# vklyukin/nf_distillation

Measured on NVIDIA B200. Metric: kd_train_samples_per_sec, higher is better.
Workload: dtype bf16

## Files before the change

### include/nfk.h

```cpp
#ifndef NFK_H_
#define NFK_H_

#ifdef __cplusplus
extern "C" {
#endif

#define NFK_OK 0
#define NFK_ERR_SHAPE (-1)
#define NFK_ERR_ALIGN (-2)
#define NFK_ERR_ARG (-3)
#define NFK_ERR_LAUNCH (-4)
#define NFK_ERR_DRIVER (-5)

#define NFK_EPI_F32 0
#define NFK_EPI_BIAS_RELU_BF16 1
#define NFK_EPI_MASK_BF16 2

int nfk_version(void);

int nfk_gemm_nt_bf16(const void* A, long long lda, const void* B, long long ldb, int M, int N, int K, int epi,
                     void* out, long long ldo, const float* bias, const void* aux, long long ldaux, float* colsum,
                     void* stream);

int nfk_gemm_set_prof(void* buf);
// ... 48 lines not shown
                      const float* l2, const float* w3, const float* b3, const float* l3, int cin, int hid, int cout,
                      int K1p, int K3p, void* B1, void* B1T, void* B2, void* B2T, void* B3, void* B3T, float* bias1,
                      float* bias2, float* bias3, int with_transposed, void* stream);

int nfk_coupling_prep_bwd(const float* w1, const float* b1, const float* l1, const float* w2, const float* b2,
                          const float* l2, const float* w3, const float* b3, const float* l3, int cin, int hid,
                          int cout, int K1p, int K3p, const float* dB1, const float* dbias1, const float* dB2,
                          const float* dbias2, const float* dB3, const float* dbias3, float* dw1, float* db1,
                          float* dl1, float* dw2, float* db2, float* dl2, float* dw3, float* db3, float* dl3,
                          void* stream);

int nfk_affine1x1_fwd(const float* x, const float* Wf, const float* bf, const float* sl, float* y, void* col,
                      int K1p, const float* ld_in, float* ld_out, int B, int C, int H, int W, void* stream);

int nfk_coupling_fwd(const float* P, int K3p, const float* bias3, float* y, float* hsave, float* ld, int B, int C,
                     int H, int W, int reverse, void* stream);

int nfk_coupling_bwd(const float* g_out, const float* g_ld, const float* z_out, const float* hsave, float* dy,
                     void* dhcol, int K3p, float* dbias3, int B, int C, int H, int W, void* stream);

int nfk_affine1x1_bwd(const float* dy, const float* dcol, int K1p, const float* x, const float* Wf, float* dx,
                      float* dWf, float* dbf, int B, int C, int H, int W, void* stream);

int nfk_coupling_inv_bwd(const float* g_zc, const float* g_ld, const float* zc, const float* hsave, float* dz,
                         void* dhcol, int K3p, float* dbias3, int B, int C, int H, int W, void* stream);

int nfk_col2im_add(const float* dcol, int K1p, float* dz, int B, int C, int H, int W, void* stream);

int nfk_split2d_fwd(const float* x, const float* w, const float* bias, const float* logs, float* z1_out, float* ld,
                    int B, int C, int H, int W, void* stream);
int nfk_split2d_rev(const float* z1, const float* w, const float* bias, const float* logs, const float* eps,
                    float temperature, float* out, int B, int C, int H, int W, void* stream);
int nfk_split2d_bwd(const float* x, const float* w, const float* bias, const float* logs, const float* g_z1,
                    const float* g_ld, float* dx, float* dw, float* dbias, float* dlogs, int B, int C, int H, int W,
                    void* stream);
int nfk_split2d_squeeze_fwd(const float* x, const float* w, const float* bias, const float* logs, float* z1_out,
                            float* z1_sq_out, float* ld, int B, int C, int H, int W, void* stream);
int nfk_split2d_squeeze_bwd(const float* x, const float* w, const float* bias, const float* logs, const float* g_z1,
                            const float* g_z1_sq, const float* g_ld, float* dx, float* dw, float* dbias, float* dlogs,
                            int B, int C, int H, int W, void* stream);
int nfk_dequant_squeeze(const void* src, int src_is_u8, int n_bits, const float* noise, float* x_out, float* sq_out,
                        int B, int C, int H, int W, void* stream);
int nfk_prior_bpd_fwd(const float* z, const float* mean, const float* logs, const float* logdet, int B, int n,
                      float scale, float* out, void* stream);
int nfk_prior_bpd_bwd(const float* z, const float* mean, const float* logs, const float* g_bpd, int B, int n,
                      float scale, float* dz, float* dlogdet, void* stream);
int nfk_kd_mse_fwd(const float* s, const float* t, int B, int n, float scale, float* acc, void* stream);
int nfk_kd_mse_bwd(const float* s, const float* t, const float* g, int B, int n, float scale, float* ds,
                   int accumulate, void* stream);

int nfk_pconv_coupling_supported(int C, int H, int W, int hid);
int nfk_pconv_coupling_fwd(const void* h2, const void* B3, int K3p, const float* bias3, float* y, float* hsave,
                           float* ld, int B, int C, int H, int W, int hid, int reverse, void* stream);

int nfk_flow1d_supported(int D, int Cc, int hid, int training);
int nfk_flow1d_sizes(int D, int Cc, int hid, int* total_fwd, int* total_bwd, int* total_grad, int* n_act,
                     int* offsets);
int nfk_flow1d_pack(const float* Wf, const float* bf, const float* const* w, const float* const* b, int D, int Cc,
                    int hid, float* PF, float* PB, void* stream);
int nfk_flow1d_fwd(const float* x, const float* cond, const float* PF, const float* sl, float* y, const float* ld_in,
                   float* ld_out, float* acts, int B, int D, int Cc, int hid, int reverse, void* stream);
int nfk_flow1d_bwd(const float* x_in, const float* cond, const float* acts, const float* PB, const float* y_out,
                   const float* g_out, const float* g_ld, float* dx, float* G, int B, int D, int Cc, int hid,
                   int reverse, void* stream);
int nfk_affine_rows(const float* x, const float* Wf, const float* bf, const float* sl, float* y, const float* ld_in,
                    float* ld_out, int B, int D, float pixels, void* stream);

int nfk_gemm_nt_bf16_ranged(const void* A, long long lda, const void* B, long long ldb, int M, int N, int K, int epi,
                            void* out, long long ldo, const float* bias, const void* aux, long long ldaux,
                            float* colsum, int bn, const int* kb_begin, const int* kb_end, void* stream);

int nfk_made_prep(const float* w1, const float* w2, const float* w3, const int* deg1, const int* deg2, int D, int H,
                  int Dp, int N3p, void* B1, void* B1T, void* B2, void* B2T, void* B3, void* B3T, int with_t,
                  void* stream);
int nfk_made_prep_bwd(const float* dB1, const float* dB2, const float* dB3, const int* deg1, const int* deg2, int D,
                      int H, int Dp, float* dw1, float* dw2, float* dw3, void* stream);
int nfk_rows_to_bf16(const float* x, int B, int D, int Dp, void* xb, void* stream);
int nfk_made_affine_fwd(const float* x, const float* out, int N3p, float* u, void* ub, int Dp, const float* ld_in,
                        float* ld_out, int B, int D, int flip, void* stream);
int nfk_made_affine_bwd(const float* x, const float* out, int N3p, const float* g_u, const float* g_ld, float* dx,
                        void* dout, float* db3, int B, int D, int flip, void* stream);
int nfk_made_inv_update(float* x, void* xb, int Dp, const float* u_in, const float* out, int N3p, const float* ld_in,
                        float* ld_out, int B, int D, int i, int flip, int last, void* stream);
int nfk_made_inverse_resident_supported(int D, int H, int Dp);
int nfk_made_inverse_push_supported(int D, int H, int Dp, int N3p);
int nfk_made_inverse_jobs(const int* cnt1, const int* cnt2, int D, int H, int Dp, int N3p, int push, int* jobs,
                          int cap);
int nfk_made_inverse_pack(const int* jobs, int njobs, const void* B1, const void* B2, const void* B3, int N3p, int D,
                          int H, int Dp, int push, void* wstream, void* stream);
int nfk_made_inverse_resident(const float* u_in, const void* wstream, const float* b1, const float* b2,
                              const float* b3, const int* jobs, int njobs, int push, int N3p, float* x,
                              const float* ld_in, float* ld_out, int B, int D, int H, int Dp, int flip, int mtiles,
                              void* stream);

int nfk_cnet_set_prof(void* buf);
int nfk_cnet_fwd_fused(const void* col, int K1p, const void* B1, const void* B2, const float* bias1,
                       const float* bias2, void* h1, void* h2, void* mask1, void* mask2, long long ldmask, int M,
                       int hid, void* stream);
int nfk_cnet_bwd_fused(const void* dhcol, int K3p, const void* B3T, const void* B2T, const void* mask_h2,
                       const void* mask_h1, long long ldmask, void* dpre2, void* dpre1, float* dbias2, float* dbias1,
                       int M, int hid, void* stream);
int nfk_cnet_fwd_fused_ranged(const void* col, int K1p, const void* B1, const void* B2, const float* bias1,
                              const float* bias2, void* h1, void* h2, void* mask1, void* mask2, long long ldmask,
                              int M, int hid, int kb2_end_half0, void* stream);

#define NFK_LOSS_MAX_LEVELS 8
// ... 37 lines not shown
```

### nf_distillation_b200/_lib.py

```python
from __future__ import annotations

import ctypes
import os

from . import build as _build

_c = ctypes
_vp, _i, _ll, _f = _c.c_void_p, _c.c_int, _c.c_longlong, _c.c_float

ERRORS = {
    -1: "NFK_ERR_SHAPE (unsupported / inconsistent sizes)",
    -2: "NFK_ERR_ALIGN (pointer or leading dimension not 16-byte aligned)",
    -3: "NFK_ERR_ARG (missing / invalid argument)",
    -4: "NFK_ERR_LAUNCH (CUDA launch failure)",
    -5: "NFK_ERR_DRIVER (tensor-map encode failure)",
}



class InvconvItem(_c.Structure):
    _fields_ = [(n, _vp) for n in ("an_bias", "an_logs", "lower", "upper", "log_s", "p", "sign_s", "weight")] + \
               [("C", _i), ("reverse", _i), ("transpose", _i)] + \
               [(n, _vp) for n in ("outW", "outb", "out_sl")]

# ... 16 lines not shown
               [(n, _vp) for n in ("dw1", "db1", "dl1", "dw2", "db2", "dl2", "dw3", "db3", "dl3")]


NFK_LOSS_MAX_LEVELS = 8


class LossLevels(_c.Structure):
    _fields_ = [("s", _vp * NFK_LOSS_MAX_LEVELS), ("t", _vp * NFK_LOSS_MAX_LEVELS), ("ds", _vp * NFK_LOSS_MAX_LEVELS),
                ("n", _i * NFK_LOSS_MAX_LEVELS), ("L", _i)]


SIGNATURES: dict[str, list] = {
    "nfk_version": [],
    "nfk_gemm_nt_bf16": [_vp, _ll, _vp, _ll, _i, _i, _i, _i, _vp, _ll, _vp, _vp, _ll, _vp, _vp],
    "nfk_gemm_set_prof": [_vp],
    "nfk_gemm_tn_bf16": [_vp, _ll, _vp, _ll, _i, _i, _i, _vp, _ll, _i, _vp],
    "nfk_invconv_prep_batch": [_i, _vp, _vp],
    "nfk_invconv_prep_bwd_batch": [_i, _vp, _vp],
    "nfk_invconv_prep": [_vp] * 8 + [_i, _i, _i, _vp, _vp, _vp, _vp],
    "nfk_invconv_prep_bwd": [_vp] * 8 + [_i, _i, _i, _vp, _vp, _vp, _vp, _i, _f] + [_vp] * 6 + [_vp],
    "nfk_coupling_prep_batch": [_i, _vp, _vp],
    "nfk_coupling_prep_bwd_batch": [_i, _vp, _vp],
    "nfk_coupling_prep": [_vp] * 9 + [_i] * 5 + [_vp] * 9 + [_i, _vp],
    "nfk_coupling_prep_bwd": [_vp] * 9 + [_i] * 5 + [_vp] * 6 + [_vp] * 9 + [_vp],
    "nfk_affine1x1_fwd": [_vp, _vp, _vp, _vp, _vp, _vp, _i, _vp, _vp, _i, _i, _i, _i, _vp],
    "nfk_coupling_fwd": [_vp, _i, _vp, _vp, _vp, _vp, _i, _i, _i, _i, _i, _vp],
    "nfk_coupling_bwd": [_vp, _vp, _vp, _vp, _vp, _vp, _i, _vp, _i, _i, _i, _i, _vp],
    "nfk_affine1x1_bwd": [_vp, _vp, _i, _vp, _vp, _vp, _vp, _vp, _i, _i, _i, _i, _vp],
    "nfk_coupling_inv_bwd": [_vp, _vp, _vp, _vp, _vp, _vp, _i, _vp, _i, _i, _i, _i, _vp],
    "nfk_col2im_add": [_vp, _i, _vp, _i, _i, _i, _i, _vp],
    "nfk_split2d_fwd": [_vp] * 6 + [_i] * 4 + [_vp],
    "nfk_split2d_rev": [_vp] * 5 + [_f, _vp] + [_i] * 4 + [_vp],
    "nfk_split2d_bwd": [_vp] * 10 + [_i] * 4 + [_vp],
    "nfk_split2d_squeeze_fwd": [_vp] * 7 + [_i] * 4 + [_vp],
    "nfk_split2d_squeeze_bwd": [_vp] * 11 + [_i] * 4 + [_vp],
    "nfk_dequant_squeeze": [_vp, _i, _i, _vp, _vp, _vp, _i, _i, _i, _i, _vp],
    "nfk_prior_bpd_fwd": [_vp] * 4 + [_i, _i, _f, _vp, _vp],
    "nfk_prior_bpd_bwd": [_vp] * 4 + [_i, _i, _f, _vp, _vp, _vp],
    "nfk_kd_mse_fwd": [_vp, _vp, _i, _i, _f, _vp, _vp],
    "nfk_kd_mse_bwd": [_vp, _vp, _vp, _i, _i, _f, _vp, _i, _vp],
    "nfk_flow1d_supported": [_i, _i, _i, _i],
    "nfk_flow1d_sizes": [_i, _i, _i, _vp, _vp, _vp, _vp, _vp],
    "nfk_flow1d_pack": [_vp, _vp, _vp, _vp, _i, _i, _i, _vp, _vp, _vp],
    "nfk_flow1d_fwd": [_vp] * 8 + [_i] * 5 + [_vp],
    "nfk_flow1d_bwd": [_vp] * 9 + [_i] * 5 + [_vp],
    "nfk_affine_rows": [_vp] * 7 + [_i, _i, _f, _vp],
    "nfk_gemm_nt_bf16_ranged": [_vp, _ll, _vp, _ll, _i, _i, _i, _i, _vp, _ll, _vp, _vp, _ll, _vp, _i, _vp, _vp, _vp],
    "nfk_cnet_set_prof": [_vp],
    "nfk_cnet_fwd_fused": [_vp, _i, _vp, _vp, _vp, _vp, _vp, _vp, _vp, _vp, _ll, _i, _i, _vp],
    "nfk_cnet_bwd_fused": [_vp, _i, _vp, _vp, _vp, _vp, _ll, _vp, _vp, _vp, _vp, _i, _i, _vp],
    "nfk_cnet_fwd_fused_ranged": [_vp, _i, _vp, _vp, _vp, _vp, _vp, _vp, _vp, _vp, _ll, _i, _i, _i, _vp],
    "nfk_pconv_coupling_supported": [_i, _i, _i, _i],
    "nfk_pconv_coupling_fwd": [_vp, _vp, _i, _vp, _vp, _vp, _vp, _i, _i, _i, _i, _i, _i, _vp],
    "nfk_made_prep": [_vp] * 5 + [_i] * 4 + [_vp] * 6 + [_i, _vp],
    "nfk_made_prep_bwd": [_vp] * 5 + [_i] * 3 + [_vp] * 3 + [_vp],
    "nfk_rows_to_bf16": [_vp, _i, _i, _i, _vp, _vp],
    "nfk_made_affine_fwd": [_vp, _vp, _i, _vp, _vp, _i, _vp, _vp, _i, _i, _i, _vp],
    "nfk_made_affine_bwd": [_vp, _vp, _i, _vp, _vp, _vp, _vp, _vp, _i, _i, _i, _vp],
    "nfk_made_inv_update": [_vp, _vp, _i, _vp, _vp, _i, _vp, _vp, _i, _i, _i, _i, _i, _vp],
    "nfk_made_inverse_resident_supported": [_i, _i, _i],
    "nfk_made_inverse_push_supported": [_i, _i, _i, _i],
    "nfk_made_inverse_jobs": [_vp, _vp, _i, _i, _i, _i, _i, _vp, _i],
    "nfk_made_inverse_pack": [_vp, _i, _vp, _vp, _vp, _i, _i, _i, _i, _i, _vp, _vp],
    "nfk_made_inverse_resident": [_vp] * 6 + [_i] * 3 + [_vp] * 3 + [_i] * 6 + [_vp],
    "nfk_kd_nll_loss_scratch_floats": [_i],
    "nfk_kd_nll_loss_fwd": [_vp, _vp, _i, _vp, _vp, _vp, _f, _vp, _vp, _vp, _f, _f, _f, _i, _vp, _vp, _vp, _vp, _vp],
    "nfk_kd_nll_loss_bwd": [_vp, _vp, _i, _vp, _vp, _f, _vp, _f, _f, _f, _i, _vp, _vp, _vp, _vp, _vp, _vp, _vp, _vp],
    "nfk_optim_partials": [],
    "nfk_grad_sqnorm": [_vp, _ll, _vp, _vp, _vp],
    "nfk_adam_step": [_vp, _vp, _vp, _vp, _ll, _vp, _vp, _f, _f, _f, _f, _f, _f, _i, _vp, _vp],
    "nfk_split3_rows": [_vp, _ll, _ll, _i, _i, _i, _vp, _vp],
    "nfk_im2col3x3_split3": [_vp, _i, _i, _i, _i, _i, _i, _i, _i, _i, _i, _vp, _vp],
    "nfk_act_split3": [_vp, _ll, _i, _i, _vp, _ll, _i, _vp, _vp, _vp],
    "nfk_coupling_bwd_f32": [_vp, _vp, _vp, _vp, _vp, _vp, _vp, _i, _i, _i, _i, _vp],
}


class NfkError(RuntimeError):
    pass


def _load() -> ctypes.CDLL:
    path = _build.LIB_PATH
    if _build.needs_build():
        try:
            _build.build()
        except Exception as e:
            if not os.path.exists(path):
                raise ImportError(
                    f"libnfk.so is not built and cannot be built here ({e}); there is no CPU fallback") from e
    lib = ctypes.CDLL(path)
    for name, argtypes in SIGNATURES.items():
        fn = getattr(lib, name)
        fn.argtypes = argtypes
        fn.restype = _c.c_int
    return lib


LIB = _load()


def check(rc: int, what: str) -> None:
    if rc != 0:
        raise NfkError(f"{what} failed: {ERRORS.get(rc, rc)}")


# ... 9 lines not shown
```

### nf_distillation_b200/csrc/pconv_coupling.cu

```cuda
#include <cuda.h>
#include <cuda_bf16.h>
#include <cuda_runtime.h>
#include <cstdint>
#include <cstdlib>

#include "../../include/nfk.h"
#include "launch_util.h"
#include "ptx.cuh"

namespace nfk {

constexpr int PC_EPI = 384;
constexpr int PC_THREADS = 64 + PC_EPI;
constexpr int PC_BK = 64;

template <int C> struct PcCfg;
template <> struct PcCfg<12> { static constexpr int NPIX = 256, MB = 1, WIN = 160, STAGES = 3; };
template <> struct PcCfg<24> { static constexpr int NPIX = 128, MB = 2, WIN = 64, STAGES = 3; };
template <> struct PcCfg<48> { static constexpr int NPIX = 64, MB = 4, WIN = 32, STAGES = 2; };

struct PcArgs {
  long long M;
  int num_kb;
  int B, H, W, lgHW, lgW;
// ... 188 lines not shown
          long long m;
          const bool live = decode(hf, et + PC_EPI * kk, j, pl, m);
          const int b = static_cast<int>(m >> g.lgHW);
          float lsum = 0.f;
          if (live) {
            const int rem = static_cast<int>(m) & HWm;
            const int yy = rem >> g.lgW, xx = rem & Wm;
            float sh = bias_s[2 * j], lg = bias_s[2 * j + 1];
            const float* sp = S + (2 * j) * Sm::pitch + (pl - w0);
#pragma unroll
            for (int tap = 0; tap < 9; ++tap) {
              const int dy = tap / 3 - 1, dx = tap % 3 - 1;
              const int ny = yy + dy, nx = xx + dx;
              if (ny >= 0 && ny < g.H && nx >= 0 && nx < g.W) {
                const float* p = sp + tap * C * Sm::pitch + dy * g.W + dx;
                sh += p[0];
                lg += p[Sm::pitch];
              }
            }
            if (g.hsave) *reinterpret_cast<float2*>(g.hsave + m * C + 2 * j) = make_float2(sh, lg);
            const float tt = lg + 2.f;
            const float e = expf(-fabsf(tt));
            const float l1p = log1pf(e);
            float sg, lsv;
            if (tt >= 0.f) { sg = 1.f / (1.f + e); lsv = -l1p; }
            else { sg = e / (1.f + e); lsv = tt - l1p; }
            g.y[((static_cast<long long>(b) * C + J + j) << g.lgHW) + rem] =
                g.reverse ? (z2v[k] / sg - sh) : (z2v[k] + sh) * sg;
            lsum = g.reverse ? -lsv : lsv;
          }
          if (g.ld) {
            const int seg = HW < 32 ? HW : 32;
#pragma unroll
            for (int o = 16; o > 0; o >>= 1) {
              const float v = __shfl_xor_sync(0xffffffffu, lsum, o);
              if (o < seg) lsum += v;
            }
            if ((lane & (seg - 1)) == 0 && live) atomicAdd(g.ld + b, lsum);
          }
        }
      }
      asm volatile("bar.sync 1, %0;" ::"n"(PC_EPI) : "memory");
    }
  }
  tc_fence_before();
  __syncthreads();
  if (warp == 1) tmem_dealloc(tmem_base, 512);
}

typedef CUresult (*EncodeTiledFn3)(CUtensorMap*, CUtensorMapDataType, cuuint32_t, void*, const cuuint64_t*,
                                   const cuuint64_t*, const cuuint32_t*, const cuuint32_t*, CUtensorMapInterleave,
                                   CUtensorMapSwizzle, CUtensorMapL2promotion, CUtensorMapFloatOOBfill);

static int pc_tmap(CUtensorMap* m, const void* ptr, uint64_t cols, uint64_t rows, uint64_t ld, uint32_t box_rows) {
  static EncodeTiledFn3 fn = nullptr;
  if (!fn) {
    void* p = nullptr;
    cudaDriverEntryPointQueryResult q;
    if (cudaGetDriverEntryPoint("cuTensorMapEncodeTiled", &p, cudaEnableDefault, &q) != cudaSuccess ||
        q != cudaDriverEntryPointSuccess)
      return NFK_ERR_DRIVER;
    fn = reinterpret_cast<EncodeTiledFn3>(p);
  }
  if ((reinterpret_cast<uintptr_t>(ptr) & 15) || (ld * 2) % 16) return NFK_ERR_ALIGN;
  cuuint64_t dims[2] = {cols, rows};
  cuuint64_t strides[1] = {ld * 2};
  cuuint32_t box[2] = {64, box_rows};
  cuuint32_t estr[2] = {1, 1};
  CUresult r = fn(m, CU_TENSOR_MAP_DATA_TYPE_BFLOAT16, 2, const_cast<void*>(ptr), dims, strides, box, estr,
                  CU_TENSOR_MAP_INTERLEAVE_NONE, CU_TENSOR_MAP_SWIZZLE_128B, CU_TENSOR_MAP_L2_PROMOTION_L2_256B,
                  CU_TENSOR_MAP_FLOAT_OOB_FILL_NONE);
  return r == CUDA_SUCCESS ? NFK_OK : NFK_ERR_DRIVER;
}

template <int C>
static int pc_launch(const void* h2, const void* B3, int K3p, const PcArgs& g, int hid, cudaStream_t st) {
  using Cfg = PcCfg<C>;
  CUtensorMap tmW, tmH;
  int rc;
  if ((rc = pc_tmap(&tmW, B3, hid, K3p, hid, 128))) return rc;
  if ((rc = pc_tmap(&tmH, h2, hid, static_cast<uint64_t>(g.M), hid, Cfg::NPIX))) return rc;
  if ((rc = ensure_dyn_smem(reinterpret_cast<const void*>(pconv_coupling_kernel<C>), PcSmem<C>::total))) return rc;
  int dev = 0, sms = 148;
  cudaGetDevice(&dev);
  cudaDeviceGetAttribute(&sms, cudaDevAttrMultiProcessorCount, dev);
  const int tiles = g.banded ? g.B * g.nb : static_cast<int>((g.M + Cfg::NPIX - 1) / Cfg::NPIX);
  const cudaError_t le = launch_pdl(pconv_coupling_kernel<C>, dim3(tiles < sms ? tiles : sms), dim3(PC_THREADS),
                                    PcSmem<C>::total, st, tmW, tmH, g);
  return (le == cudaSuccess && cudaGetLastError() == cudaSuccess) ? NFK_OK : NFK_ERR_LAUNCH;
}

int pconv_px_launch(const void* h2, const void* B3, int K3p, const float* bias3, float* y, float* hsave, float* ld,
                    int B, int C, int hid, int reverse, cudaStream_t st);
static bool pconv_use_px() {
  static const bool v = [] { const char* e = getenv("NFK_PCONV_PX"); return !(e && e[0] == '0'); }();
  return v;
}

}

using namespace nfk;

extern "C" int nfk_pconv_coupling_supported(int C, int H, int W, int hid) {
  if (hid <= 0 || hid % 64) return 0;
  const int HW = H * W;
  if (HW < 4 || (HW & (HW - 1)) || (W & (W - 1))) return 0;
  if (C == 12) {
// ... 36 lines not shown
```

### nf_distillation_b200/functional.py

```python
from __future__ import annotations

import os
from dataclasses import dataclass
from typing import Optional

import torch

from . import ops

BF16 = torch.bfloat16
F32 = torch.float32
USE_FUSED_CNET = os.environ.get("NFK_FUSED_CNET", "1") != "0"
USE_FUSED_PCONV = os.environ.get("NFK_FUSED_PCONV", "1") != "0"
USE_FUSED_CNET_BWD = os.environ.get("NFK_FUSED_CNET_BWD", "1") != "0"

WGRAD_STREAM_MAX_M = int(os.environ.get("NFK_WGRAD_STREAM_MAX_M", "65536"))
_wgrad_streams: dict = {}
_wgrad_keepalive: list = []


def _wgrad_stream(dev):
    key = (dev.type, dev.index if dev.index is not None else torch.cuda.current_device())
    st = _wgrad_streams.get(key)
    if st is None:
        st = _wgrad_streams[key] = torch.cuda.Stream(device=dev)
    return st


def _join_wgrads(dev):
    if _wgrad_keepalive:
        torch.cuda.current_stream(dev).wait_stream(_wgrad_stream(dev))
        _wgrad_keepalive.clear()

_PARAM_EPOCH = [0]


def bump_param_epoch() -> None:
    _PARAM_EPOCH[0] += 1


def param_key(params) -> tuple:
    params = list(params)
    epoch = _PARAM_EPOCH[0] if any(p.requires_grad for p in params) else -1
    return (epoch, tuple((p.data_ptr(), p._version) for p in params))


@dataclass
class StepConsts:
    Wf: torch.Tensor
    bf: torch.Tensor
    sl: torch.Tensor
    B1: torch.Tensor = None
    B1T: torch.Tensor = None
    B2: torch.Tensor = None
    B2T: torch.Tensor = None
    B3: torch.Tensor = None
    B3T: torch.Tensor = None
    bias1: torch.Tensor = None
    bias2: torch.Tensor = None
    bias3: torch.Tensor = None


def build_affine(an_bias, an_logs, inv, C, reverse, transpose):
    dev = an_bias.device
    Wf = torch.empty(C, C, device=dev, dtype=F32)
    bf = torch.empty(C, device=dev, dtype=F32)
    sl = torch.empty(1, device=dev, dtype=F32)
# ... 233 lines not shown
    _conv3_coupling(h2, k, y, hsave, ld_out, B, C, H, W, hid, K3p, False)
    return y, ld_out, (col, h1, h2 if keep else None, hsave, m1, m2)


def flowstep2d_reverse(z, ld_in, k: StepConsts, hid, keep=False):
    B, C, H, W = z.shape
    M, cin = B * H * W, C // 2
    K1p, K3p = ops.round_up(9 * cin, 64), ops.round_up(9 * C, 64)
    dev = z.device
    col = torch.empty(M, K1p, device=dev, dtype=BF16)
    ops.affine1x1_fwd(z, None, None, None, None, col, K1p, None, None, B, C, H, W)
    h1, h2, m1, m2 = _coupling_net(col, k, M, hid, K1p, K3p, keep)
    hsave = torch.empty(M, C, device=dev, dtype=F32) if keep else None
    zc = z.clone()
    ld_mid = ld_in.clone()
    _conv3_coupling(h2, k, zc, hsave, ld_mid, B, C, H, W, hid, K3p, True)
    x = torch.empty_like(z)
    ld_out = torch.empty_like(ld_mid)
    ops.affine1x1_fwd(zc, k.Wf, k.bf, k.sl, x, None, 0, ld_mid, ld_out, B, C, H, W)
    if keep:
        return x, ld_out, (zc, col, h1, h2, hsave, m1, m2)
    return x, ld_out


def _grad_arena(C, hid, K1p, K3p, dev):
    sizes = [C, hid, hid, K3p * hid, hid * hid, hid * K1p, C * C, C]
    offs = [0]
    for s in sizes:
        offs.append(offs[-1] + ops.round_up(s, 4))
    arena = torch.zeros(offs[-1], device=dev, dtype=F32)
    dbias3, dbias2, dbias1, dB3, dB2, dB1, dWf, dbf = (arena[offs[i]:offs[i] + sizes[i]] for i in range(8))
    return (arena, dbias3, dbias2, dbias1, dB3.view(K3p, hid), dB2.view(hid, hid), dB1.view(hid, K1p),
            dWf.view(C, C), dbf)


def _coupling_net_backward(dhcol, col, h1, h2, m1, m2, B1T, B2T, B3T, dbias2, dbias1, dB3, dB2, dB1, arena, M, hid,
                           K1p, K3p):
    dev = dhcol.device
    dpre2 = torch.empty(M, hid, device=dev, dtype=BF16)
    dpre1 = torch.empty(M, hid, device=dev, dtype=BF16)
    if USE_FUSED_CNET_BWD and ops.cnet_fused_supported(hid, K3p) and M >= 8192:
        ops.cnet_bwd_fused(dhcol, K3p, B3T, B2T, m2, m1, dpre2, dpre1, dbias2, dbias1, M, hid)
    else:
        ops.gemm_nt(dhcol, B3T, M, hid, K3p, ops.EPI_MASK_BF16, dpre2, aux=m2, colsum=dbias2)
        ops.gemm_nt(dpre2, B2T, M, hid, hid, ops.EPI_MASK_BF16, dpre1, aux=m1, colsum=dbias1)
    if 0 < M <= WGRAD_STREAM_MAX_M:
        cur, side = torch.cuda.current_stream(dev), _wgrad_stream(dev)
        side.wait_stream(cur)
        with torch.cuda.stream(side):
            ops.gemm_tn(dhcol, h2, K3p, hid, M, dB3)
            ops.gemm_tn(dpre2, h1, hid, hid, M, dB2)
            ops.gemm_tn(dpre1, col, hid, K1p, M, dB1)
        _wgrad_keepalive.append((dhcol, dpre2, dpre1, h1, h2, col, arena))
        dcol = torch.empty(M, K1p, device=dev, dtype=F32)
        ops.gemm_nt(dpre1, B1T, M, K1p, hid, ops.EPI_F32, dcol)
    else:
        ops.gemm_tn(dhcol, h2, K3p, hid, M, dB3)
        ops.gemm_tn(dpre2, h1, hid, hid, M, dB2)
        dcol = torch.empty(M, K1p, device=dev, dtype=F32)
        ops.gemm_nt(dpre1, B1T, M, K1p, hid, ops.EPI_F32, dcol)
        ops.gemm_tn(dpre1, col, hid, K1p, M, dB1)
    return dcol


class FlowStep2dFn(torch.autograd.Function):

    @staticmethod
    def forward(ctx, x, ld_in, hid, token, pctx, idx):
        B, C, H, W = x.shape
        x = x.contiguous()
        Wf, bf, sl = pctx.consts[idx]
        k = StepConsts(Wf, bf, sl, *pctx.cops[idx])
        y, ld_out, (col, h1, h2, hsave, m1, m2) = flowstep2d_forward(x, ld_in.contiguous(), k, hid, keep=True)
        ctx.hid = hid
        ctx.pctx, ctx.idx = pctx, idx
        ctx.save_for_backward(x, y, col, h1, h2, hsave, m1, m2, Wf, k.B1T, k.B2T, k.B3T)
        return y, ld_out

    @staticmethod
    def backward(ctx, g_out, g_ld):
        (x, z_out, col, h1, h2, hsave, m1, m2, Wf, B1T, B2T, B3T) = ctx.saved_tensors
        hid = ctx.hid
        B, C, H, W = x.shape
        M, cin = B * H * W, C // 2
        K1p, K3p = ops.round_up(9 * cin, 64), ops.round_up(9 * C, 64)
        dev = x.device
        _join_wgrads(dev)
        g_out = torch.zeros_like(x) if g_out is None else g_out.contiguous()
        g_ld = torch.zeros(B, device=dev, dtype=F32) if g_ld is None else g_ld.contiguous()
        arena, dbias3, dbias2, dbias1, dB3, dB2, dB1, dWf, dbf = _grad_arena(C, hid, K1p, K3p, dev)

        dy = torch.empty_like(x)
        dhcol = torch.empty(M, K3p, device=dev, dtype=BF16)
        ops.coupling_bwd(g_out, g_ld, z_out, hsave, dy, dhcol, K3p, dbias3, B, C, H, W)
        dcol = _coupling_net_backward(dhcol, col, h1, h2, m1, m2, B1T, B2T, B3T, dbias2, dbias1, dB3, dB2, dB1, arena,
                                      M, hid, K1p, K3p)
        dx = torch.empty_like(x)
        ops.affine1x1_bwd(dy, dcol, K1p, x, Wf, dx, dWf, dbf, B, C, H, W)

        ctx.pctx.grads[ctx.idx] = (dWf, C, dbf, g_ld, B, float(H * W))
        ctx.pctx.cgrads[ctx.idx] = (dB1, dbias1, dB2, dbias2, dB3, dbias3)
        return (dx, g_ld, None, None, None, None)


class FlowStep2dReverseFn(torch.autograd.Function):

    @staticmethod
    def forward(ctx, z, ld_in, hid, token, pctx, idx):
        z = z.contiguous()
        Wf, bf, sl = pctx.consts[idx]
        k = StepConsts(Wf, bf, sl, *pctx.cops[idx])
        x, ld_out, (zc, col, h1, h2, hsave, m1, m2) = flowstep2d_reverse(z, ld_in.contiguous(), k, hid, keep=True)
        ctx.hid = hid
        ctx.pctx, ctx.idx = pctx, idx
        ctx.save_for_backward(zc, col, h1, h2, hsave, m1, m2, Wf, k.B1T, k.B2T, k.B3T)
        return x, ld_out

    @staticmethod
    def backward(ctx, g_x, g_ld):
        (zc, col, h1, h2, hsave, m1, m2, Wf, B1T, B2T, B3T) = ctx.saved_tensors
        hid = ctx.hid
        B, C, H, W = zc.shape
        M, cin = B * H * W, C // 2
        K1p, K3p = ops.round_up(9 * cin, 64), ops.round_up(9 * C, 64)
        dev = zc.device
        _join_wgrads(dev)
        g_x = torch.zeros_like(zc) if g_x is None else g_x.contiguous()
        g_ld = torch.zeros(B, device=dev, dtype=F32) if g_ld is None else g_ld.contiguous()
        arena, dbias3, dbias2, dbias1, dB3, dB2, dB1, dWf, dbf = _grad_arena(C, hid, K1p, K3p, dev)

        dzc = torch.empty_like(zc)
        ops.affine1x1_bwd(g_x, None, K1p, zc, Wf, dzc, dWf, dbf, B, C, H, W)
        dz = torch.empty_like(zc)
        dhcol = torch.empty(M, K3p, device=dev, dtype=BF16)
        ops.coupling_inv_bwd(dzc, g_ld, zc, hsave, dz, dhcol, K3p, dbias3, B, C, H, W)
        dcol = _coupling_net_backward(dhcol, col, h1, h2, m1, m2, B1T, B2T, B3T, dbias2, dbias1, dB3, dB2, dB1, arena,
                                      M, hid, K1p, K3p)
        ops.col2im_add(dcol, K1p, dz, B, C, H, W)

        ctx.pctx.grads[ctx.idx] = (dWf, C, dbf, g_ld, B, float(H * W))
        ctx.pctx.cgrads[ctx.idx] = (dB1, dbias1, dB2, dbias2, dB3, dbias3)
        return (dz, g_ld, None, None, None, None)


class Split2dFn(torch.autograd.Function):
    @staticmethod
    def forward(ctx, x, ld_in, w, bias, logs):
        B, C, H, W = x.shape
        x = x.contiguous()
        z1 = torch.empty(B, C // 2, H, W, device=x.device, dtype=F32)
        ld = ld_in.clone()
        ops.split2d_fwd(x, w, bias, logs, z1, ld, B, C, H, W)
        ctx.save_for_backward(x, w, bias, logs)
        return z1, ld

    @staticmethod
    def backward(ctx, g_z1, g_ld):
        x, w, bias, logs = ctx.saved_tensors
        B, C, H, W = x.shape
        dev = x.device
        g_ld = torch.zeros(B, device=dev, dtype=F32) if g_ld is None else g_ld.contiguous()
        g_z1 = None if g_z1 is None else g_z1.contiguous()
        dx = torch.empty_like(x)
        nw = w.numel()
        arena = torch.zeros(nw + 2 * C, device=dev, dtype=F32)
        dw, dbias, dlogs = arena[:nw].view_as(w), arena[nw:nw + C].view_as(bias), arena[nw + C:].view_as(logs)
        ops.split2d_bwd(x, w, bias, logs, g_z1, g_ld, dx, dw, dbias, dlogs, B, C, H, W)
        return dx, g_ld, dw, dbias, dlogs


class Split2dSqueezeFn(torch.autograd.Function):

    @staticmethod
    def forward(ctx, x, ld_in, w, bias, logs):
        B, C, H, W = x.shape
        x = x.contiguous()
        z1 = torch.empty(B, C // 2, H, W, device=x.device, dtype=F32)
        z1_sq = torch.empty(B, 2 * C, H // 2, W // 2, device=x.device, dtype=F32)
        ld = ld_in.clone()
        ops.split2d_fwd(x, w, bias, logs, z1, ld, B, C, H, W, z1_sq=z1_sq)
        ctx.save_for_backward(x, w, bias, logs)
        return z1, z1_sq, ld

    @staticmethod
    def backward(ctx, g_z1, g_sq, g_ld):
        x, w, bias, logs = ctx.saved_tensors
        B, C, H, W = x.shape
        dev = x.device
        g_ld = torch.zeros(B, device=dev, dtype=F32) if g_ld is None else g_ld.contiguous()
        g_z1 = None if g_z1 is None else g_z1.contiguous()
        g_sq = None if g_sq is None else g_sq.contiguous()
# ... 132 lines not shown
```

### nf_distillation_b200/ops.py

```python
from __future__ import annotations

import ctypes

import torch

from ._lib import LIB, check

EPI_F32, EPI_BIAS_RELU_BF16, EPI_MASK_BF16 = 0, 1, 2

_LAUNCHES = 0


def launch_count() -> int:
    return _LAUNCHES


def _p(t):
    if t is None:
        return None
    assert t.is_cuda and t.is_contiguous(), "libnfk needs contiguous CUDA tensors"
    return t.data_ptr()


def _st():
# ... 178 lines not shown
                                      _st()), "nfk_split2d_squeeze_fwd")


def dequant_squeeze(src, noise, x_out, sq_out, n_bits=8):
    _count()
    B, C, H, W = src.shape
    check(LIB.nfk_dequant_squeeze(_p(src), int(src.dtype == torch.uint8), n_bits, _p(noise), _p(x_out), _p(sq_out),
                                  B, C, H, W, _st()), "nfk_dequant_squeeze")


def split2d_rev(z1, w, bias, logs, eps, temperature, out, B, C, H, W):
    _count()
    check(LIB.nfk_split2d_rev(_p(z1), _p(w), _p(bias), _p(logs), _p(eps), float(temperature), _p(out), B, C, H, W,
                              _st()), "nfk_split2d_rev")


def split2d_bwd(x, w, bias, logs, g_z1, g_ld, dx, dw, dbias, dlogs, B, C, H, W, g_z1_sq=None):
    _count()
    check(LIB.nfk_split2d_squeeze_bwd(_p(x), _p(w), _p(bias), _p(logs), _p(g_z1), _p(g_z1_sq), _p(g_ld), _p(dx),
                                      _p(dw), _p(dbias), _p(dlogs), B, C, H, W, _st()), "nfk_split2d_squeeze_bwd")


def prior_bpd_fwd(z, mean, logs, logdet, B, n, scale, out):
    _count()
    check(LIB.nfk_prior_bpd_fwd(_p(z), _p(mean), _p(logs), _p(logdet), B, n, float(scale), _p(out), _st()),
          "nfk_prior_bpd_fwd")


def prior_bpd_bwd(z, mean, logs, g_bpd, B, n, scale, dz, dlogdet):
    _count()
    check(LIB.nfk_prior_bpd_bwd(_p(z), _p(mean), _p(logs), _p(g_bpd), B, n, float(scale), _p(dz), _p(dlogdet),
                                _st()), "nfk_prior_bpd_bwd")


def kd_mse_fwd(s, t, B, n, scale, acc):
    _count()
    check(LIB.nfk_kd_mse_fwd(_p(s), _p(t), B, n, float(scale), _p(acc), _st()), "nfk_kd_mse_fwd")


def kd_mse_bwd(s, t, g, B, n, scale, ds, accumulate=False):
    _count()
    check(LIB.nfk_kd_mse_bwd(_p(s), _p(t), _p(g), B, n, float(scale), _p(ds), int(accumulate), _st()),
          "nfk_kd_mse_bwd")


def pconv_coupling_supported(C, H, W, hid):
    return bool(LIB.nfk_pconv_coupling_supported(C, H, W, hid))


def pconv_coupling_fwd(h2, B3, K3p, bias3, y, hsave, ld, B, C, H, W, hid, reverse):
    _count()
    check(LIB.nfk_pconv_coupling_fwd(_p(h2), _p(B3), K3p, _p(bias3), _p(y), _p(hsave), _p(ld), B, C, H, W, hid,
                                     int(reverse), _st()), "nfk_pconv_coupling_fwd")


def flow1d_supported(D, Cc, hid, training=False):
    return bool(LIB.nfk_flow1d_supported(D, Cc, hid, int(training)))


def flow1d_sizes(D, Cc, hid):
    import ctypes
    vals = [ctypes.c_int() for _ in range(4)]
    offs = (ctypes.c_int * 28)()
    check(LIB.nfk_flow1d_sizes(D, Cc, hid, *[ctypes.addressof(v) for v in vals], ctypes.addressof(offs)),
          "nfk_flow1d_sizes")
    return (*[v.value for v in vals], [tuple(offs[4 * l:4 * l + 4]) for l in range(7)])


def flow1d_pack(Wf, bf, ws, bs, D, Cc, hid, PF, PB):
    import ctypes
    _count()
    wa = (ctypes.c_void_p * 6)(*[_p(t) for t in ws])
    ba = (ctypes.c_void_p * 6)(*[_p(t) for t in bs])
    check(LIB.nfk_flow1d_pack(_p(Wf), _p(bf), ctypes.addressof(wa), ctypes.addressof(ba), D, Cc, hid, _p(PF), _p(PB),
                              _st()), "nfk_flow1d_pack")


def flow1d_fwd(x, cond, PF, sl, y, ld_in, ld_out, acts, B, D, Cc, hid, reverse):
    _count()
    check(LIB.nfk_flow1d_fwd(_p(x), _p(cond), _p(PF), _p(sl), _p(y), _p(ld_in), _p(ld_out), _p(acts), B, D, Cc, hid,
                             int(reverse), _st()), "nfk_flow1d_fwd")


def flow1d_bwd(x_in, cond, acts, PB, y_out, g_out, g_ld, dx, G, B, D, Cc, hid, reverse):
    _count()
    check(LIB.nfk_flow1d_bwd(_p(x_in), _p(cond), _p(acts), _p(PB), _p(y_out), _p(g_out), _p(g_ld), _p(dx), _p(G), B, D,
                             Cc, hid, int(reverse), _st()), "nfk_flow1d_bwd")


def affine_rows(x, Wf, bf, sl, y, ld_in, ld_out, B, D, pixels):
    _count()
    check(LIB.nfk_affine_rows(_p(x), _p(Wf), _p(bf), _p(sl), _p(y), _p(ld_in), _p(ld_out), B, D, float(pixels),
                              _st()), "nfk_affine_rows")


def gemm_nt_ranged(A, B, M, N, K, epi, out, bn, kb_begin, kb_end, bias=None, aux=None, colsum=None):
    import ctypes
    _count()
    n = len(kb_begin)
    kb0 = (ctypes.c_int * n)(*kb_begin)
    kb1 = (ctypes.c_int * n)(*kb_end)
    check(LIB.nfk_gemm_nt_bf16_ranged(_p(A), A.stride(0), _p(B), B.stride(0), M, N, K, epi, _p(out), out.stride(0),
                                      _p(bias), _p(aux), 0 if aux is None else aux.stride(0), _p(colsum), bn,
                                      ctypes.addressof(kb0), ctypes.addressof(kb1), _st()), "nfk_gemm_nt_bf16_ranged")


# ... 140 lines not shown
```

Before: 53690.

## Fuse conv1 data-gradient GEMM with col2im and affine 1x1 backward

Adds a tcgen05/TMA kernel that computes the first coupling-conv data gradient (dpre1 x B1T) into tensor memory, then performs col2im, the 1x1 invertible-conv backward (dx, dWf, dbf) in an epilogue from shared memory. This replaces a separate GEMM writing an fp32 dcol buffer plus a separate affine1x1_bwd kernel for the forward-direction coupling path, avoiding the dcol round trip through global memory and one launch. It is limited to C in {12,24,48} with power-of-two spatial sizes and uses atomics for weight-gradient reduction across CTAs. The reverse path keeps the old GEMM plus col2im.

```diff
diff --git a/include/nfk.h b/include/nfk.h
--- a/include/nfk.h
+++ b/include/nfk.h
@@ -124,6 +124,11 @@
 int nfk_pconv_coupling_supported(int C, int H, int W, int hid);
 int nfk_pconv_coupling_fwd(const void* h2, const void* B3, int K3p, const float* bias3, float* y, float* hsave,
                            float* ld, int B, int C, int H, int W, int hid, int reverse, void* stream);
+
+int nfk_conv1_dgrad_affine_bwd_supported(int C, int H, int W, int hid);
+int nfk_conv1_dgrad_affine_bwd(const void* dpre1, const void* B1T, int K1p, const float* dy, const float* x,
+                               const float* Wf, float* dx, float* dWf, float* dbf, int B, int C, int H, int W, int hid,
+                               void* stream);
 
 int nfk_flow1d_supported(int D, int Cc, int hid, int training);
 int nfk_flow1d_sizes(int D, int Cc, int hid, int* total_fwd, int* total_bwd, int* total_grad, int* n_act,
diff --git a/nf_distillation_b200/_lib.py b/nf_distillation_b200/_lib.py
--- a/nf_distillation_b200/_lib.py
+++ b/nf_distillation_b200/_lib.py
@@ -92,6 +92,8 @@
     "nfk_cnet_fwd_fused_ranged": [_vp, _i, _vp, _vp, _vp, _vp, _vp, _vp, _vp, _vp, _ll, _i, _i, _i, _vp],
     "nfk_pconv_coupling_supported": [_i, _i, _i, _i],
     "nfk_pconv_coupling_fwd": [_vp, _vp, _i, _vp, _vp, _vp, _vp, _i, _i, _i, _i, _i, _i, _vp],
+    "nfk_conv1_dgrad_affine_bwd_supported": [_i, _i, _i, _i],
+    "nfk_conv1_dgrad_affine_bwd": [_vp] * 9 + [_i] * 5 + [_vp],
     "nfk_made_prep": [_vp] * 5 + [_i] * 4 + [_vp] * 6 + [_i, _vp],
     "nfk_made_prep_bwd": [_vp] * 5 + [_i] * 3 + [_vp] * 3 + [_vp],
     "nfk_rows_to_bf16": [_vp, _i, _i, _i, _vp, _vp],
diff --git a/nf_distillation_b200/csrc/dgrad_col2im.cu b/nf_distillation_b200/csrc/dgrad_col2im.cu
--- /dev/null
+++ b/nf_distillation_b200/csrc/dgrad_col2im.cu
@@ -0,0 +1,374 @@
+#include <cuda.h>
+#include <cuda_bf16.h>
+#include <cuda_runtime.h>
+#include <cstdint>
+
+#include "../../include/nfk.h"
+#include "launch_util.h"
+#include "ptx.cuh"
+
+namespace nfk {
+
+constexpr int DG_EPI = 256;
+constexpr int DG_THREADS = 64 + DG_EPI;
+constexpr int DG_BK = 64;
+
+template <int C> struct DgCfg;
+template <> struct DgCfg<12> { static constexpr int NPIX = 256, MB = 1, STAGES = 3; };
+template <> struct DgCfg<24> { static constexpr int NPIX = 128, MB = 1, STAGES = 4; };
+template <> struct DgCfg<48> { static constexpr int NPIX = 64, MB = 2, STAGES = 3; };
+
+struct DgArgs {
+  int B, lgHW, lgW, H, W;
+  int num_kb;
+  int a_box_rows;
+  const float* dy;
+  const float* x;
+  const float* Wf;
+  float* dx;
+  float* dWf;
+  float* dbf;
+};
+
+template <int C>
+struct DgSmem {
+  using Cfg = DgCfg<C>;
+  static constexpr int a_bytes = Cfg::MB * 128 * 128;
+  static constexpr int b_bytes = Cfg::NPIX * 128;
+  static constexpr int stage_bytes = a_bytes + b_bytes;
+  static constexpr int pitch = Cfg::NPIX + 1;
+  static constexpr int s_bytes = ((9 * (C / 2) * pitch * 4 + 15) / 16) * 16;
+  static constexpr int t_bytes = C * pitch * 4;
+  static constexpr int off_s = Cfg::STAGES * stage_bytes;
+  static constexpr int off_dys = off_s + s_bytes;
+  static constexpr int off_xs = off_dys + t_bytes;
+  static constexpr int off_wt = off_xs + t_bytes;
+  static constexpr int off_acc = off_wt + C * C * 4;
+  static constexpr int off_bar = off_acc + ((C * 4 + 15) / 16) * 16;
+  static constexpr int total = off_bar + 128;
+  static_assert(total <= 227 * 1024, "shared memory budget");
+};
+
+template <int C>
+__global__ void __launch_bounds__(DG_THREADS, 1)
+conv1_dgrad_affine_bwd_kernel(const __grid_constant__ CUtensorMap tmW, const __grid_constant__ CUtensorMap tmD,
+                              const DgArgs g) {
+  using Cfg = DgCfg<C>;
+  using Sm = DgSmem<C>;
+  constexpr int NPIX = Cfg::NPIX, MB = Cfg::MB, STAGES = Cfg::STAGES;
+  constexpr int CH = C / 2, K1 = 9 * CH;
+  constexpr int ACC_COLS = MB * NPIX;
+  constexpr int TMEM_COLS = 2 * ACC_COLS;
+  constexpr int ldp = Sm::pitch;
+  extern __shared__ __align__(1024) uint8_t smem[];
+  pdl_launch_dependents();
+  if (smem_u32(smem) & 1023u) __trap();
+  const int warp = static_cast<int>(uniform_u32(threadIdx.x >> 5)), lane = threadIdx.x & 31;
+  float* S = reinterpret_cast<float*>(smem + Sm::off_s);
+  float* dys = reinterpret_cast<float*>(smem + Sm::off_dys);
+  float* xs = reinterpret_cast<float*>(smem + Sm::off_xs);
+  float* WT = reinterpret_cast<float*>(smem + Sm::off_wt);
+  float* acc = reinterpret_cast<float*>(smem + Sm::off_acc);
+  uint64_t* full = reinterpret_cast<uint64_t*>(smem + Sm::off_bar);
+  uint64_t* empty = full + STAGES;
+  uint64_t* tmem_full = empty + STAGES;
+  uint64_t* tmem_empty = tmem_full + 2;
+  uint32_t* tmem_slot = reinterpret_cast<uint32_t*>(tmem_empty + 2);
+
+  const int ipt = NPIX >> g.lgHW;
+  const int num_tiles = (g.B + ipt - 1) / ipt;
+  if (warp == 0 && lane == 0) {
+    tma_prefetch_desc(&tmW);
+    tma_prefetch_desc(&tmD);
+    for (int s = 0; s < STAGES; ++s) { mbar_init(&full[s], 1); mbar_init(&empty[s], 1); }
+    for (int a = 0; a < 2; ++a) { mbar_init(&tmem_full[a], 1); mbar_init(&tmem_empty[a], 8); }
+    fence_mbar_init();
+  }
+  if (warp == 1) { tmem_alloc(tmem_slot, TMEM_COLS); tmem_relinquish(); }
+  pdl_wait();
+  tc_fence_before();
+  __syncthreads();
+  tc_fence_after();
+  const uint32_t tmem_base = uniform_u32(*tmem_slot);
+
+  if (warp == 0) {
+    {
+      const uint32_t tx = MB * g.a_box_rows * 128 + Sm::b_bytes;
+      int s = 0;
+      uint32_t ph = 0;
+      for (int t = blockIdx.x; t < num_tiles; t += gridDim.x) {
+        for (int kb = 0; kb < g.num_kb; ++kb) {
+          mbar_wait_warp(&empty[s], ph ^ 1);
+          uint8_t* sa = smem + s * Sm::stage_bytes;
+          mbar_expect_tx_elect(&full[s], tx);
+#pragma unroll
+          for (int mb = 0; mb < MB; ++mb) tma_load_2d_elect(sa + mb * 128 * 128, &tmW, &full[s], kb * DG_BK, mb * 128);
+          tma_load_2d_elect(sa + Sm::a_bytes, &tmD, &full[s], kb * DG_BK, t * NPIX);
+          if (++s == STAGES) { s = 0; ph ^= 1; }
+        }
+      }
+    }
+  } else if (warp == 1) {
+    {
+      const uint32_t idesc = umma_idesc_bf16(128, NPIX, false, false);
+      int s = 0, it = 0;
+      uint32_t ph = 0;
+      for (int t = blockIdx.x; t < num_tiles; t += gridDim.x, ++it) {
+        const int ac = it & 1;
+        mbar_wait_warp(&tmem_empty[ac], ((it >> 1) & 1) ^ 1);
+        tc_fence_after();
+        const uint32_t tmem_d = tmem_base + ac * ACC_COLS;
+        for (int kb = 0; kb < g.num_kb; ++kb) {
+          mbar_wait_warp(&full[s], ph);
+          tc_fence_after();
+          const uint32_t a_addr = smem_u32(smem + s * Sm::stage_bytes);
+          const uint32_t b_addr = a_addr + Sm::a_bytes;
+#pragma unroll
+          for (int k = 0; k < DG_BK / 16; ++k) {
+            const uint64_t bd = umma_desc_sw128(b_addr + k * 32, 16, 1024);
+#pragma unroll
+            for (int mb = 0; mb < MB; ++mb) {
+              const uint64_t ad = umma_desc_sw128(a_addr + mb * 128 * 128 + k * 32, 16, 1024);
+              umma_f16_elect(tmem_d + mb * NPIX, ad, bd, idesc, (kb > 0 || k > 0) ? 1u : 0u);
+            }
+          }
+          umma_commit_elect(&empty[s]);
+          if (++s == STAGES) { s = 0; ph ^= 1; }
+        }
+        umma_commit_elect(&tmem_full[ac]);
+      }
+    }
+  } else {
+    const int q = warp & 3, half = (warp - 2) >> 2;
+    const int et = threadIdx.x - 64;
+    const int HW = 1 << g.lgHW, HWm = HW - 1, Wm = g.W - 1;
+    for (int i = et; i < C * C; i += DG_EPI) {
+      const int o = i / C, c = i - o * C;
+      WT[c * C + o] = g.Wf[i];
+    }
+    for (int i = et; i < C; i += DG_EPI) acc[i] = 0.f;
+    constexpr int NBK = (C / 4) * (C / 4);
+    constexpr int SL = NBK >= DG_EPI ? 1 : DG_EPI / NBK;
+    static_assert(NBK <= DG_EPI, "one dW' block per thread");
+    float wacc[4][4] = {};
+    constexpr int PARTS = DG_EPI / NPIX;
+    static_assert(DG_EPI % NPIX == 0 && C % (4 * PARTS) == 0, "dx split");
+    constexpr int ITEMS = CH * NPIX / DG_EPI;
+    static_assert(CH * NPIX % DG_EPI == 0, "col2im items divide over the epilogue threads");
+    constexpr int TLD = C * NPIX / DG_EPI;
+    static_assert(C * NPIX % DG_EPI == 0, "tile loads divide over the epilogue threads");
+
+    float xv[TLD], dv[TLD];
+    auto load_tile = [&](int t) {
+      const int b0 = t * ipt;
+      const int nel = (min(ipt, g.B - b0) * C) << g.lgHW;
+      const long long base = static_cast<long long>(b0) * C << g.lgHW;
+#pragma unroll
+      for (int u = 0; u < TLD; ++u) {
+        const int i = et + u * DG_EPI;
+        xv[u] = i < nel ? __ldg(g.x + base + i) : 0.f;
+        dv[u] = i < nel ? __ldg(g.dy + base + i) : 0.f;
+      }
+    };
+    if (static_cast<int>(blockIdx.x) < num_tiles) load_tile(blockIdx.x);
+
+    int it = 0;
+    for (int t = blockIdx.x; t < num_tiles; t += gridDim.x, ++it) {
+      const int ac = it & 1;
+      const int b0 = t * ipt;
+      const int npix = min(ipt, g.B - b0) << g.lgHW;
+#pragma unroll
+      for (int u = 0; u < TLD; ++u) {
+        const int i = et + u * DG_EPI;
+        const int ic = i >> g.lgHW, img = ic / C, c = ic - img * C;
+        const int so = c * ldp + (img << g.lgHW) + (i & HWm);
+        xs[so] = xv[u];
+        dys[so] = dv[u];
+      }
+      if (t + static_cast<int>(gridDim.x) < num_tiles) load_tile(t + gridDim.x);
+      mbar_wait(&tmem_full[ac], (it >> 1) & 1);
+      tc_fence_after();
+      {
+        constexpr int HCOLS = NPIX / 2;
+        static_assert(HCOLS % 32 == 0, "column halves are drained 32 columns at a time");
+#pragma unroll
+        for (int mb = 0; mb < MB; ++mb) {
+          const int row = mb * 128 + q * 32 + lane;
+          const uint32_t taddr = tmem_base + (static_cast<uint32_t>(q * 32) << 16) + ac * ACC_COLS + mb * NPIX +
+                                 half * HCOLS;
+          float* srow = S + row * ldp + half * HCOLS;
+          if (mb * 128 + q * 32 < K1) {
+#pragma unroll 1
+            for (int c = 0; c < HCOLS; c += 32) {
+              uint32_t r0[16], r1[16];
+              tmem_ld16(taddr + c, r0);
+              tmem_ld16(taddr + c + 16, r1);
+              tmem_ld_wait();
+              if (row < K1) {
+#pragma unroll
+                for (int k = 0; k < 16; ++k) srow[c + k] = __uint_as_float(r0[k]);
+#pragma unroll
+                for (int k = 0; k < 16; ++k) srow[c + 16 + k] = __uint_as_float(r1[k]);
+              }
+            }
+          }
+        }
+        tc_fence_before();
+        __syncwarp();
+        if (lane == 0) mbar_arrive(&tmem_empty[ac]);
+      }
+      asm volatile("bar.sync 1, %0;" ::"n"(DG_EPI) : "memory");
+#pragma unroll
+      for (int u = 0; u < ITEMS; ++u) {
+        const int i = et + u * DG_EPI;
+        const int ci = i / NPIX, pl = i % NPIX;
+        if (pl < npix) {
+          const int rem = pl & HWm;
+          const int yy = rem >> g.lgW, xx = rem & Wm;
+          const float* sp = S + ci * ldp + pl;
+          float a = 0.f;
+#pragma unroll
+          for (int tap = 0; tap < 9; ++tap) {
+            const int ddy = tap / 3 - 1, ddx = tap % 3 - 1;
+            const int ny = yy - ddy, nx = xx - ddx;
+            a += (ny >= 0 && ny < g.H && nx >= 0 && nx < g.W) ? sp[tap * CH * ldp - ddy * g.W - ddx] : 0.f;
+          }
+          dys[ci * ldp + pl] += a;
+        }
+      }
+      asm volatile("bar.sync 1, %0;" ::"n"(DG_EPI) : "memory");
+      {
+        const int pl = et % NPIX, part = et / NPIX;
+        if (pl < npix) {
+          const int img = pl >> g.lgHW, rem = pl & HWm;
+          float dv[C];
+#pragma unroll
+          for (int o = 0; o < C; ++o) dv[o] = dys[o * ldp + pl];
+          float* dxp = g.dx + ((static_cast<long long>(b0 + img) * C) << g.lgHW) + rem;
+#pragma unroll 2
+          for (int ii = 0; ii < C / PARTS; ++ii) {
+            const int i = part * (C / PARTS) + ii;
+            float a = 0.f;
+            const float4* wr = reinterpret_cast<const float4*>(WT + i * C);
+#pragma unroll
+            for (int o = 0; o < C / 4; ++o) {
+              const float4 w = wr[o];
+              a = fmaf(w.x, dv[4 * o], a);
+              a = fmaf(w.y, dv[4 * o + 1], a);
+              a = fmaf(w.z, dv[4 * o + 2], a);
+              a = fmaf(w.w, dv[4 * o + 3], a);
+            }
+            dxp[static_cast<long long>(i) << g.lgHW] = a;
+          }
+        }
+      }
+      {
+        const int blk = et % NBK, slice = et / NBK;
+        if (slice < SL) {
+          const int to = blk / (C / 4), ti = blk % (C / 4);
+#pragma unroll 4
+          for (int p = slice; p < npix; p += SL) {
+            float dw[4], xw[4];
+#pragma unroll
+            for (int qq = 0; qq < 4; ++qq) {
+              dw[qq] = dys[(4 * to + qq) * ldp + p];
+              xw[qq] = xs[(4 * ti + qq) * ldp + p];
+            }
+#pragma unroll
+            for (int qq = 0; qq < 4; ++qq)
+#pragma unroll
+              for (int r = 0; r < 4; ++r) wacc[qq][r] = fmaf(dw[qq], xw[r], wacc[qq][r]);
+          }
+        }
+      }
+      {
+        const int ew = et >> 5;
+        for (int o = ew; o < C; o += DG_EPI / 32) {
+          float a = 0.f;
+          for (int p = lane; p < npix; p += 32) a += dys[o * ldp + p];
+          for (int sft = 16; sft > 0; sft >>= 1) a += __shfl_xor_sync(0xffffffffu, a, sft);
+          if (lane == 0) acc[o] += a;
+        }
+      }
+      asm volatile("bar.sync 1, %0;" ::"n"(DG_EPI) : "memory");
+    }
+    static_assert(SL * C * C * 4 <= Sm::s_bytes, "slice scratch fits in S");
+    {
+      const int blk = et % NBK, slice = et / NBK;
+      if (slice < SL) {
+        const int to = blk / (C / 4), ti = blk % (C / 4);
+#pragma unroll
+        for (int qq = 0; qq < 4; ++qq)
+#pragma unroll
+          for (int r = 0; r < 4; ++r) S[slice * C * C + (4 * to + qq) * C + 4 * ti + r] = wacc[qq][r];
+      }
+    }
+    asm volatile("bar.sync 1, %0;" ::"n"(DG_EPI) : "memory");
+    for (int i = et; i < C * C; i += DG_EPI) {
+      float a = 0.f;
+      for (int sl2 = 0; sl2 < SL; ++sl2) a += S[sl2 * C * C + i];
+      atomicAdd(g.dWf + i, a);
+    }
+    for (int i = et; i < C; i += DG_EPI) atomicAdd(g.dbf + i, acc[i]);
+  }
+  tc_fence_before();
+  __syncthreads();
+  if (warp == 1) tmem_dealloc(tmem_base, TMEM_COLS);
+}
+
+int pc_tmap(CUtensorMap* m, const void* ptr, uint64_t cols, uint64_t rows, uint64_t ld, uint32_t box_rows);
+
+template <int C>
+static int dg_launch(const void* dpre1, const void* B1T, int K1p, int hid, DgArgs g, cudaStream_t st) {
+  using Cfg = DgCfg<C>;
+  CUtensorMap tmW, tmD;
+  int rc;
+  g.a_box_rows = K1p < 128 ? K1p : 128;
+  const long long M = static_cast<long long>(g.B) << g.lgHW;
+  if ((rc = pc_tmap(&tmW, B1T, hid, K1p, hid, g.a_box_rows))) return rc;
+  if ((rc = pc_tmap(&tmD, dpre1, hid, static_cast<uint64_t>(M), hid, Cfg::NPIX))) return rc;
+  if ((rc = ensure_dyn_smem(reinterpret_cast<const void*>(conv1_dgrad_affine_bwd_kernel<C>), DgSmem<C>::total)))
+    return rc;
+  int dev = 0, sms = 148;
+  cudaGetDevice(&dev);
+  cudaDeviceGetAttribute(&sms, cudaDevAttrMultiProcessorCount, dev);
+  const int ipt = Cfg::NPIX >> g.lgHW;
+  const int tiles = (g.B + ipt - 1) / ipt;
+  const cudaError_t le = launch_pdl(conv1_dgrad_affine_bwd_kernel<C>, dim3(tiles < sms ? tiles : sms),
+                                    dim3(DG_THREADS), DgSmem<C>::total, st, tmW, tmD, g);
+  return (le == cudaSuccess && cudaGetLastError() == cudaSuccess) ? NFK_OK : NFK_ERR_LAUNCH;
+}
+
+}
+
+using namespace nfk;
+
+extern "C" int nfk_conv1_dgrad_affine_bwd_supported(int C, int H, int W, int hid) {
+  if (hid <= 0 || hid % 64) return 0;
+  if (H <= 0 || W <= 0 || (H & (H - 1)) || (W & (W - 1))) return 0;
+  const int HW = H * W;
+  switch (C) {
+    case 12: return HW <= DgCfg<12>::NPIX;
+    case 24: return HW <= DgCfg<24>::NPIX;
+    case 48: return HW <= DgCfg<48>::NPIX;
+    default: return 0;
+  }
+}
+
+extern "C" int nfk_conv1_dgrad_affine_bwd(const void* dpre1, const void* B1T, int K1p, const float* dy,
+                                          const float* x, const float* Wf, float* dx, float* dWf, float* dbf, int B,
+                                          int C, int H, int W, int hid, void* stream) {
+  if (B <= 0 || !nfk_conv1_dgrad_affine_bwd_supported(C, H, W, hid)) return NFK_ERR_SHAPE;
+  if (K1p != (9 * (C / 2) + 63) / 64 * 64) return NFK_ERR_SHAPE;
+  if (!dpre1 || !B1T || !dy || !x || !Wf || !dx || !dWf || !dbf) return NFK_ERR_ARG;
+  DgArgs g{};
+  g.B = B; g.H = H; g.W = W;
+  g.lgW = 0; while ((1 << g.lgW) < W) ++g.lgW;
+  g.lgHW = 0; while ((1 << g.lgHW) < H * W) ++g.lgHW;
+  g.num_kb = hid / 64;
+  g.dy = dy; g.x = x; g.Wf = Wf; g.dx = dx; g.dWf = dWf; g.dbf = dbf;
+  cudaStream_t st = static_cast<cudaStream_t>(stream);
+  if (C == 12) return dg_launch<12>(dpre1, B1T, K1p, hid, g, st);
+  if (C == 24) return dg_launch<24>(dpre1, B1T, K1p, hid, g, st);
+  return dg_launch<48>(dpre1, B1T, K1p, hid, g, st);
+}
diff --git a/nf_distillation_b200/csrc/pconv_coupling.cu b/nf_distillation_b200/csrc/pconv_coupling.cu
--- a/nf_distillation_b200/csrc/pconv_coupling.cu
+++ b/nf_distillation_b200/csrc/pconv_coupling.cu
@@ -264,7 +264,7 @@
                                    const cuuint64_t*, const cuuint32_t*, const cuuint32_t*, CUtensorMapInterleave,
                                    CUtensorMapSwizzle, CUtensorMapL2promotion, CUtensorMapFloatOOBfill);
 
-static int pc_tmap(CUtensorMap* m, const void* ptr, uint64_t cols, uint64_t rows, uint64_t ld, uint32_t box_rows) {
+int pc_tmap(CUtensorMap* m, const void* ptr, uint64_t cols, uint64_t rows, uint64_t ld, uint32_t box_rows) {
   static EncodeTiledFn3 fn = nullptr;
   if (!fn) {
     void* p = nullptr;
diff --git a/nf_distillation_b200/functional.py b/nf_distillation_b200/functional.py
--- a/nf_distillation_b200/functional.py
+++ b/nf_distillation_b200/functional.py
@@ -13,6 +13,7 @@
 USE_FUSED_CNET = os.environ.get("NFK_FUSED_CNET", "1") != "0"
 USE_FUSED_PCONV = os.environ.get("NFK_FUSED_PCONV", "1") != "0"
 USE_FUSED_CNET_BWD = os.environ.get("NFK_FUSED_CNET_BWD", "1") != "0"
+USE_FUSED_DGRAD1 = os.environ.get("NFK_FUSED_DGRAD1", "1") != "0"
 
 WGRAD_STREAM_MAX_M = int(os.environ.get("NFK_WGRAD_STREAM_MAX_M", "65536"))
 _wgrad_streams: dict = {}
@@ -352,14 +353,16 @@
             ops.gemm_tn(dpre2, h1, hid, hid, M, dB2)
             ops.gemm_tn(dpre1, col, hid, K1p, M, dB1)
         _wgrad_keepalive.append((dhcol, dpre2, dpre1, h1, h2, col, arena))
-        dcol = torch.empty(M, K1p, device=dev, dtype=F32)
-        ops.gemm_nt(dpre1, B1T, M, K1p, hid, ops.EPI_F32, dcol)
     else:
         ops.gemm_tn(dhcol, h2, K3p, hid, M, dB3)
         ops.gemm_tn(dpre2, h1, hid, hid, M, dB2)
-        dcol = torch.empty(M, K1p, device=dev, dtype=F32)
-        ops.gemm_nt(dpre1, B1T, M, K1p, hid, ops.EPI_F32, dcol)
         ops.gemm_tn(dpre1, col, hid, K1p, M, dB1)
+    return dpre1
+
+
+def _conv1_dgrad(dpre1, B1T, M, K1p, hid):
+    dcol = torch.empty(M, K1p, device=dpre1.device, dtype=F32)
+    ops.gemm_nt(dpre1, B1T, M, K1p, hid, ops.EPI_F32, dcol)
     return dcol
 
 
@@ -393,10 +396,14 @@
         dy = torch.empty_like(x)
         dhcol = torch.empty(M, K3p, device=dev, dtype=BF16)
         ops.coupling_bwd(g_out, g_ld, z_out, hsave, dy, dhcol, K3p, dbias3, B, C, H, W)
-        dcol = _coupling_net_backward(dhcol, col, h1, h2, m1, m2, B1T, B2T, B3T, dbias2, dbias1, dB3, dB2, dB1, arena,
-                                      M, hid, K1p, K3p)
+        dpre1 = _coupling_net_backward(dhcol, col, h1, h2, m1, m2, B1T, B2T, B3T, dbias2, dbias1, dB3, dB2, dB1, arena,
+                                       M, hid, K1p, K3p)
         dx = torch.empty_like(x)
-        ops.affine1x1_bwd(dy, dcol, K1p, x, Wf, dx, dWf, dbf, B, C, H, W)
+        if USE_FUSED_DGRAD1 and ops.conv1_dgrad_affine_bwd_supported(C, H, W, hid):
+            ops.conv1_dgrad_affine_bwd(dpre1, B1T, K1p, dy, x, Wf, dx, dWf, dbf, B, C, H, W, hid)
+        else:
+            dcol = _conv1_dgrad(dpre1, B1T, M, K1p, hid)
+            ops.affine1x1_bwd(dy, dcol, K1p, x, Wf, dx, dWf, dbf, B, C, H, W)
 
         ctx.pctx.grads[ctx.idx] = (dWf, C, dbf, g_ld, B, float(H * W))
         ctx.pctx.cgrads[ctx.idx] = (dB1, dbias1, dB2, dbias2, dB3, dbias3)
@@ -434,9 +441,9 @@
         dz = torch.empty_like(zc)
         dhcol = torch.empty(M, K3p, device=dev, dtype=BF16)
         ops.coupling_inv_bwd(dzc, g_ld, zc, hsave, dz, dhcol, K3p, dbias3, B, C, H, W)
-        dcol = _coupling_net_backward(dhcol, col, h1, h2, m1, m2, B1T, B2T, B3T, dbias2, dbias1, dB3, dB2, dB1, arena,
-                                      M, hid, K1p, K3p)
-        ops.col2im_add(dcol, K1p, dz, B, C, H, W)
+        dpre1 = _coupling_net_backward(dhcol, col, h1, h2, m1, m2, B1T, B2T, B3T, dbias2, dbias1, dB3, dB2, dB1, arena,
+                                       M, hid, K1p, K3p)
+        ops.col2im_add(_conv1_dgrad(dpre1, B1T, M, K1p, hid), K1p, dz, B, C, H, W)
 
         ctx.pctx.grads[ctx.idx] = (dWf, C, dbf, g_ld, B, float(H * W))
         ctx.pctx.cgrads[ctx.idx] = (dB1, dbias1, dB2, dbias2, dB3, dbias3)
diff --git a/nf_distillation_b200/ops.py b/nf_distillation_b200/ops.py
--- a/nf_distillation_b200/ops.py
+++ b/nf_distillation_b200/ops.py
@@ -254,6 +254,17 @@
     _count()
     check(LIB.nfk_pconv_coupling_fwd(_p(h2), _p(B3), K3p, _p(bias3), _p(y), _p(hsave), _p(ld), B, C, H, W, hid,
                                      int(reverse), _st()), "nfk_pconv_coupling_fwd")
+
+
+def conv1_dgrad_affine_bwd_supported(C, H, W, hid):
+    return bool(LIB.nfk_conv1_dgrad_affine_bwd_supported(C, H, W, hid))
+
+
+def conv1_dgrad_affine_bwd(dpre1, B1T, K1p, dy, x, Wf, dx, dWf, dbf, B, C, H, W, hid):
+    assert dpre1.dtype == torch.bfloat16 and B1T.dtype == torch.bfloat16
+    _count()
+    check(LIB.nfk_conv1_dgrad_affine_bwd(_p(dpre1), _p(B1T), K1p, _p(dy), _p(x), _p(Wf), _p(dx), _p(dWf), _p(dbf), B,
+                                         C, H, W, hid, _st()), "nfk_conv1_dgrad_affine_bwd")
 
 
 def flow1d_supported(D, Cc, hid, training=False):
```

Result: faster. 55410, median of 6 (+3.2%).
